# eora-ai/torchok

Hardware: AMD Instinct MI355X
Metric: images/sec (node) ResNet-50 224px bs256/GPU; step p50 ms (higher is better)
Workload: dtype bf16

## Files before the change

### torchok_amd/csrc/pw_gemm.hip

```cpp
#include "pw_gemm.h"
#include <stdlib.h>

namespace {

constexpr int BK = 64;
constexpr int BM = 128;

__device__ __forceinline__ int fw_swz(int n) {
  return ((0x78 >> (((n >> 3) & 3) << 1)) & 3) | (((n >> 1) & 1) << 2);
}

struct PwDiv { uint32_t mul, shift; };
PwDiv make_pwdiv(uint32_t d) {
  PwDiv f = {0, 0};
  if (d <= 1) return f;
  uint32_t l = 0;
  while ((1ull << l) < d) ++l;
  f.mul = (uint32_t)((((1ull << 32) * ((1ull << l) - d)) / d) + 1);
  f.shift = l;
  return f;
}
__device__ __forceinline__ uint32_t pwdiv(uint32_t n, PwDiv f) { return (uint32_t)(((uint64_t)__umulhi(n, f.mul) + n) >> f.shift); }

__device__ __forceinline__ u32x4 lds_read16(uint32_t addr) {
  u32x4 v;
  asm volatile("ds_read_b128 %0, %1" : "=v"(v) : "v"(addr));
  return v;
}
__device__ __forceinline__ uint32_t lds_read_u8(uint32_t addr) {
  uint32_t v;
  asm volatile("ds_read_u8 %0, %1" : "=v"(v) : "v"(addr));
  return v;
}

template <int BN, bool BNEP>
__global__ __launch_bounds__(256, BN == 64 ? 2 : 1) void pw_gemm_ring_kernel(PwArgs a, uint32_t x_bytes, uint32_t w_bytes,
                                                                             uint32_t y_bytes, uint32_t m_bytes, int KT,
                                                                             int SPT, uint32_t e1_bytes, PwDiv fd_hw, PwDiv fd_w,
                                                                             uint32_t x2_bytes, uint32_t w2_bytes, int KT1) {
  constexpr int NT = 256;
  constexpr int WGN = BN / 64;
  constexpr int WGM = (NT / 64) / WGN;
  constexpr int MT = BM / (WGM * 16);
  constexpr int RSTEP = NT / 8;
  constexpr int AROWS = BM / RSTEP;
  constexpr int WROWS = BN / RSTEP;
  constexpr int A_BYTES = BM * BK * 2;
  constexpr int W_BYTES = BN * BK * 2;
  constexpr int MK_BYTES = BN == 64 ? 1024 : 4096;
  constexpr int STAGE = A_BYTES + W_BYTES + MK_BYTES;
  constexpr int LOADS = AROWS + WROWS + 1;
  constexpr int NST = 3;

  extern __shared__ __attribute__((aligned(16))) char smem[];
  typedef __attribute__((address_space(3))) char lds_char;
  typedef __attribute__((address_space(3))) void lds_void;
  const uint32_t lds_base = (uint32_t)(size_t)(lds_char*)smem;

  const int tid = threadIdx.x;
  const int lane = tid & 63;
  const int wv = tid >> 6;
  const int wn = wv % WGN;
  const int wm = wv / WGN;
  const int kc = tid & 7;
  const int lrow = tid >> 3;
  const int kcA = kc ^ (lrow & 7);
  const int kcW = kc ^ fw_swz(lrow);
  const int wave_u = __builtin_amdgcn_readfirstlane(tid >> 6);

  const __amdgpu_buffer_rsrc_t xsrd = __builtin_amdgcn_make_buffer_rsrc((void*)a.x, 0, x_bytes, 0x00020000);
  const __amdgpu_buffer_rsrc_t wsrd = __builtin_amdgcn_make_buffer_rsrc((void*)a.w, 0, w_bytes, 0x00020000);
  const __amdgpu_buffer_rsrc_t x2srd = __builtin_amdgcn_make_buffer_rsrc((void*)(a.x2 ? a.x2 : a.x), 0, a.x2 ? x2_bytes : 0, 0x00020000);
  const __amdgpu_buffer_rsrc_t w2srd = __builtin_amdgcn_make_buffer_rsrc((void*)(a.w2 ? a.w2 : a.w), 0, a.w2 ? w2_bytes : 0, 0x00020000);
  const __amdgpu_buffer_rsrc_t e1srd = __builtin_amdgcn_make_buffer_rsrc((void*)(a.e1 ? a.e1 : a.x), 0, a.e1 ? e1_bytes : 0, 0x00020000);
  const __amdgpu_buffer_rsrc_t e2srd = __builtin_amdgcn_make_buffer_rsrc((void*)(a.e2 ? a.e2 : a.x), 0, a.e2 ? y_bytes : 0, 0x00020000);
  const __amdgpu_buffer_rsrc_t msrd =
      __builtin_amdgcn_make_buffer_rsrc((void*)(a.mask_in ? (const void*)a.mask_in : (const void*)a.x), 0, a.mask_in ? m_bytes : 0, 0x00020000);

  const int xcd = blockIdx.x & 7, jx = blockIdx.x >> 3;
  const int bn_fixed = jx % a.gridN, jm = jx / a.gridN;
  const int S8 = (gridDim.x >> 3) / a.gridN;
  const int sweep = 8 * S8;
  const int n0 = bn_fixed * BN;
  const int it0 = xcd * S8 + jm;
  const int ntiles = it0 < a.gridM ? (a.gridM - it0 + sweep - 1) / sweep : 0;
  const int total = ntiles * SPT;
  const int nE1 = a.e1 != nullptr ? 1 : 0;
  const int mask_cols = a.N >> 3;

  int itL = it0, ksL = 0;
  auto issue = [&](int slot) {
    char* Adst = smem + slot * STAGE + wave_u * 1024;
    char* Wdst = smem + slot * STAGE + A_BYTES + wave_u * 1024;
    char* Mdst = smem + slot * STAGE + A_BYTES + W_BYTES + wave_u * (MK_BYTES / 4);
    const bool live = itL < a.gridM;
    const int m0 = itL * BM;
    const bool kstage = ksL < KT;
    const bool last = ksL == SPT - 1;
    if (kstage) {
      const bool second = ksL >= KT1;
      const int kl = second ? ksL - KT1 : ksL;
      const int Cc = second ? a.C2 : a.C;
      const __amdgpu_buffer_rsrc_t xs = second ? x2srd : xsrd;
      const __amdgpu_buffer_rsrc_t ws = second ? w2srd : wsrd;
      const int kcol = kl * BK + kcA * 8;
#pragma unroll
      for (int i = 0; i < AROWS; ++i) {
        const int m = m0 + lrow + RSTEP * i;
        uint32_t off = (live && m < a.M && kcol < Cc) ? (uint32_t)(m * Cc + kcol) * 2u : 0xFFFFFFF0u;
        asm volatile("" : "+v"(off));
        __builtin_amdgcn_raw_ptr_buffer_load_lds(xs, (lds_void*)(Adst + i * (RSTEP * 128)), 16, off, 0, 0, 0);
      }
      const int wcol = kl * BK + kcW * 8;
#pragma unroll
      for (int j = 0; j < WROWS; ++j) {
        const int n = n0 + lrow + RSTEP * j;
        uint32_t off = (live && n < a.N && wcol < Cc) ? (uint32_t)(n * Cc + wcol) * 2u : 0xFFFFFFF0u;
        asm volatile("" : "+v"(off));
        __builtin_amdgcn_raw_ptr_buffer_load_lds(ws, (lds_void*)(Wdst + j * (RSTEP * 128)), 16, off, 0, 0, 0);
      }
    } else {
      const bool first_e = (ksL - KT) == 0 && nE1;
      const __amdgpu_buffer_rsrc_t esrd = first_e ? e1srd : e2srd;
      const bool sub = first_e && a.e1_sub;
      auto erow = [&](int m, int n, bool ok) -> uint32_t {
        if (!ok) return 0xFFFFFFF0u;
        if (sub) {
          const uint32_t b = pwdiv((uint32_t)m, fd_hw);
          const uint32_t rem = (uint32_t)m - b * (uint32_t)(a.sub_H * a.sub_W);
          const uint32_t h = pwdiv(rem, fd_w);
          const uint32_t w = rem - h * (uint32_t)a.sub_W;
          if ((h | w) & 1u) return 0xFFFFFFF0u;
          const uint32_t ph = (uint32_t)(a.sub_H + 1) >> 1, pw = (uint32_t)(a.sub_W + 1) >> 1;
          return (((b * ph + (h >> 1)) * pw + (w >> 1)) * (uint32_t)a.N + (uint32_t)n) * 2u;
        }
        return (uint32_t)(m * a.N + n) * 2u;
      };
#pragma unroll
      for (int i = 0; i < AROWS; ++i) {
        const int m = m0 + lrow + RSTEP * i;
        const int n = n0 + kcA * 8;
        uint32_t off = erow(m, n, live && m < a.M && n < a.N);
        asm volatile("" : "+v"(off));
        __builtin_amdgcn_raw_ptr_buffer_load_lds(esrd, (lds_void*)(Adst + i * (RSTEP * 128)), 16, off, 0, 0, 0);
      }
#pragma unroll
      for (int j = 0; j < WROWS; ++j) {
        const int m = m0 + lrow + RSTEP * j;
        const int n = n0 + 64 + kcA * 8;
        uint32_t off = erow(m, n, BN == 128 && live && m < a.M && n < a.N);
        asm volatile("" : "+v"(off));
        __builtin_amdgcn_raw_ptr_buffer_load_lds(esrd, (lds_void*)(Wdst + j * (RSTEP * 128)), 16, off, 0, 0, 0);
      }
    }
    {
      uint32_t off = 0xFFFFFFF0u;
      if (BN == 64) {
        const int row = tid >> 1;
        if (live && last && a.mask_in != nullptr && m0 + row < a.M) off = (uint32_t)((m0 + row) * mask_cols + (n0 >> 3) + (tid & 1) * 4);
        asm volatile("" : "+v"(off));
        __builtin_amdgcn_raw_ptr_buffer_load_lds(msrd, (lds_void*)Mdst, 4, off, 0, 0, 0);
      } else {
        if (live && last && a.mask_in != nullptr && tid < BM && m0 + tid < a.M) off = (uint32_t)((m0 + tid) * mask_cols + (n0 >> 3));
        asm volatile("" : "+v"(off));
        __builtin_amdgcn_raw_ptr_buffer_load_lds(msrd, (lds_void*)Mdst, 16, off, 0, 0, 0);
      }
    }
    if (++ksL == SPT) { ksL = 0; itL += sweep; }
  };

  const int sl = lane >> 4;
  const int li = lane & 15;
  const int wrow0 = wn * 64 + (li >> 2) * 8 + (li & 3);
  const int wswz = fw_swz(wrow0);
  const int arow0 = wm * (MT * 16) + li;
  const int aswz = li & 7;

  float s1[16], s2[16];
#pragma unroll
  for (int c = 0; c < 16; ++c) { s1[c] = 0.f; s2[c] = 0.f; }
  float esc[16], esh[16];
  if (BNEP) {
#pragma unroll
    for (int c = 0; c < 16; ++c) {
      const int n = n0 + wn * 64 + sl * 8 + (c >> 3) * 32 + (c & 7);
      esc[c] = n < a.N ? a.ep_scale[n] : 0.f;
      esh[c] = n < a.N ? a.ep_shift[n] : 0.f;
    }
  }
  float bia[16];
#pragma unroll
  for (int c = 0; c < 16; ++c) {
    const int n = n0 + wn * 64 + sl * 8 + (c >> 3) * 32 + (c & 7);
    bia[c] = (a.bias != nullptr && n < a.N) ? a.bias[n] : 0.f;
  }

  f32x4 acc[4][MT];
  auto zero_acc = [&]() {
#pragma unroll
    for (int t = 0; t < 4; ++t)
#pragma unroll
      for (int mt = 0; mt < MT; ++mt) acc[t][mt] = (f32x4){0.f, 0.f, 0.f, 0.f};
  };

  auto compute = [&](uint32_t sb) {
    const uint32_t Ab = sb, Wb = sb + A_BYTES;
    u32x4 wf[2][4], af[2][MT];
#pragma unroll
    for (int kk = 0; kk < 2; ++kk) {
      const int s = sl + 4 * kk;
#pragma unroll
      for (int t = 0; t < 4; ++t) wf[kk][t] = lds_read16(Wb + (wrow0 + (t >> 1) * 32 + (t & 1) * 4) * 128 + ((s ^ wswz) << 4));
#pragma unroll
      for (int mt = 0; mt < MT; ++mt) af[kk][mt] = lds_read16(Ab + (arow0 + mt * 16) * 128 + ((s ^ aswz) << 4));
    }
    asm volatile("s_waitcnt lgkmcnt(%0)" ::"n"(4 + MT) : "memory");
    __builtin_amdgcn_sched_barrier(0);
#pragma unroll
    for (int t = 0; t < 4; ++t)
#pragma unroll
      for (int mt = 0; mt < MT; ++mt)
        acc[t][mt] = __builtin_amdgcn_mfma_f32_16x16x32_bf16(__builtin_bit_cast(bf16x8, wf[0][t]), __builtin_bit_cast(bf16x8, af[0][mt]),
                                                             acc[t][mt], 0, 0, 0);
    __builtin_amdgcn_sched_barrier(0);
    asm volatile("s_waitcnt lgkmcnt(0)" ::: "memory");
    __builtin_amdgcn_sched_barrier(0);
#pragma unroll
    for (int t = 0; t < 4; ++t)
#pragma unroll
      for (int mt = 0; mt < MT; ++mt)
        acc[t][mt] = __builtin_amdgcn_mfma_f32_16x16x32_bf16(__builtin_bit_cast(bf16x8, wf[1][t]), __builtin_bit_cast(bf16x8, af[1][mt]),
                                                             acc[t][mt], 0, 0, 0);
  };

  auto etile = [&](uint32_t sb, bf16x8 (&dst)[MT][2]) {
    u32x4 raw[MT][2];
#pragma unroll
    for (int mt = 0; mt < MT; ++mt)
#pragma unroll
      for (int half = 0; half < 2; ++half)
        raw[mt][half] = lds_read16(sb + wn * A_BYTES + (arow0 + mt * 16) * 128 + (((sl + 4 * half) ^ aswz) << 4));
    asm volatile("s_waitcnt lgkmcnt(0)" ::: "memory");
    __builtin_amdgcn_sched_barrier(0);
#pragma unroll
    for (int mt = 0; mt < MT; ++mt)
#pragma unroll
      for (int half = 0; half < 2; ++half) dst[mt][half] = __builtin_bit_cast(bf16x8, raw[mt][half]);
  };

  auto add_e1 = [&](uint32_t sb) {
    bf16x8 ev[MT][2];
    etile(sb, ev);
#pragma unroll
    for (int mt = 0; mt < MT; ++mt)
#pragma unroll
      for (int half = 0; half < 2; ++half)
#pragma unroll
        for (int e = 0; e < 8; ++e) acc[half * 2 + (e >> 2)][mt][e & 3] += bf2f(ev[mt][half][e]);
  };

  auto epilogue = [&](int it, uint32_t sb) {
    const int m0 = it * BM;
    const int nb = n0 + wn * 64 + sl * 8;
    bf16x8 ev[MT][2];
    const bool need_tile = BNEP ? (a.e1 != nullptr) : (a.e2 != nullptr);
    if (need_tile) etile(sb, ev);
    uint32_t mbits[MT][2];
    if (a.mask_in != nullptr) {
#pragma unroll
      for (int mt = 0; mt < MT; ++mt)
#pragma unroll
        for (int half = 0; half < 2; ++half)
          mbits[mt][half] = lds_read_u8(sb + A_BYTES + W_BYTES + (arow0 + mt * 16) * (BN / 8) + wn * 8 + sl + half * 4);
      asm volatile("s_waitcnt lgkmcnt(0)" ::: "memory");
      __builtin_amdgcn_sched_barrier(0);
    }
#pragma unroll
    for (int mt = 0; mt < MT; ++mt) {
      const int m = m0 + arow0 + mt * 16;
      if (m >= a.M) continue;
      bf16* yp = a.y + (size_t)m * a.N + nb;
#pragma unroll
      for (int half = 0; half < 2; ++half) {
        if (nb + half * 32 + 8 > a.N) continue;
        float v[8];
#pragma unroll
        for (int e = 0; e < 8; ++e) v[e] = acc[half * 2 + (e >> 2)][mt][e & 3] + bia[half * 8 + e];
        bf16x8 o;
#pragma unroll
        for (int e = 0; e < 8; ++e) o[e] = f2bf(v[e]);
        const size_t eoff = (size_t)m * a.N + nb + half * 32;
        if (BNEP) {
          unsigned bits = 0;
#pragma unroll
          for (int e = 0; e < 8; ++e) {
            float z = fmaf(v[e], esc[half * 8 + e], esh[half * 8 + e]);
            if (a.e1 != nullptr) z += bf2f(ev[mt][half][e]);
            if (a.ep_relu) z = fmaxf(z, 0.f);
            o[e] = f2bf(z);
            bits |= (bf2f(o[e]) > 0.f ? 1u : 0u) << e;
          }
          if (a.mask_out != nullptr) a.mask_out[eoff >> 3] = (uint8_t)bits;
        }
        if (a.mask_store) {
          const unsigned bits = mbits[mt][half];
#pragma unroll
          for (int e = 0; e < 8; ++e) {
            if (!((bits >> e) & 1u)) o[e] = (bf16)0.f;
            s1[half * 8 + e] += bf2f(o[e]);
          }
        }
        stg16(yp + half * 32, o);
        if (a.stats != nullptr && !a.mask_store) {
          if (a.e2 != nullptr) {
            const unsigned bits = a.mask_in != nullptr ? mbits[mt][half] : 0xffu;
#pragma unroll
            for (int e = 0; e < 8; ++e) {
              const float dz = ((bits >> e) & 1u) ? bf2f(o[e]) : 0.f;
              s1[half * 8 + e] += dz;
              s2[half * 8 + e] = fmaf(dz, bf2f(ev[mt][half][e]), s2[half * 8 + e]);
            }
          } else {
#pragma unroll
            for (int e = 0; e < 8; ++e) {
              const float r = bf2f(o[e]);
              s1[half * 8 + e] += r;
              s2[half * 8 + e] = fmaf(r, r, s2[half * 8 + e]);
            }
          }
        }
      }
    }
  };

  zero_acc();
  issue(0);
  issue(1);
  int cur = 0, nxt = 2;
  int itC = it0, ksC = 0;
  for (int s = 0; s < total; ++s) {
    asm volatile("s_waitcnt vmcnt(%0) lgkmcnt(0)" ::"n"(LOADS) : "memory");
    __builtin_amdgcn_s_barrier();
    issue(nxt);
    const uint32_t sb = lds_base + cur * STAGE;
    if (ksC < KT) {
      compute(sb);
    } else if (!BNEP && a.accumulate && ksC == KT) {
      add_e1(sb);
    }
    if (ksC == SPT - 1) {
      epilogue(itC, sb);
      zero_acc();
      ksC = 0;
      itC += sweep;
    } else {
      ++ksC;
    }
    cur = cur == NST - 1 ? 0 : cur + 1;
    nxt = nxt == NST - 1 ? 0 : nxt + 1;
  }
  asm volatile("s_waitcnt vmcnt(0) lgkmcnt(0)" ::: "memory");

  if (a.stats != nullptr) {
    __syncthreads();
    float* red = reinterpret_cast<float*>(smem);
#pragma unroll
    for (int step = 0; step < 4; ++step) {
      const int off = 8 >> step;
      const int cnt = 8 >> step;
      const bool up = (li & off) != 0;
#pragma unroll
      for (int j = 0; j < cnt; ++j) {
        const float send1 = up ? s1[j] : s1[j + cnt];
        const float send2 = up ? s2[j] : s2[j + cnt];
        const float keep1 = up ? s1[j + cnt] : s1[j];
        const float keep2 = up ? s2[j + cnt] : s2[j];
        s1[j] = keep1 + __shfl_xor(send1, off, 64);
        s2[j] = keep2 + __shfl_xor(send2, off, 64);
      }
    }
    const int nl = wn * 64 + (li >> 3) * 32 + sl * 8 + (li & 7);
    red[(0 * WGM + wm) * BN + nl] = s1[0];
    red[(1 * WGM + wm) * BN + nl] = s2[0];
    __syncthreads();
    if (tid < 2 * BN) {
      const int which = tid / BN;
      const int c = tid - which * BN;
      float t = 0.f;
#pragma unroll
      for (int w_ = 0; w_ < WGM; ++w_) t += red[(which * WGM + w_) * BN + c];
      const int row = xcd * S8 + jm;
      const int n = n0 + c;
      if (n < a.N) a.stats[((size_t)which * a.stat_rows + row) * a.N + n] = t;
    }
  }
}

template <int BN, bool BNEP>
int launch_ring(const PwArgs& a, hipStream_t st) {
  constexpr int STAGE = BM * BK * 2 + BN * BK * 2 + (BN == 64 ? 1024 : 4096);
  constexpr int smem = 3 * STAGE;
  static const bool attr_set = [&] {
    (void)hipFuncSetAttribute(reinterpret_cast<const void*>(&pw_gemm_ring_kernel<BN, BNEP>),
                              hipFuncAttributeMaxDynamicSharedMemorySize, smem);
    return true;
  }();
  (void)attr_set;
  const int KT1 = tok_cdiv(a.C, BK);
  const int KT = KT1 + (a.x2 != nullptr ? tok_cdiv(a.C2, BK) : 0);
  const int SPT = KT + (a.e1 ? 1 : 0) + (a.e2 ? 1 : 0);
  const unsigned long long xb = (unsigned long long)a.M * a.C * 2, wb = (unsigned long long)a.N * a.C * 2,
                           yb = (unsigned long long)a.M * a.N * 2, mb = (unsigned long long)a.M * (a.N / 8);
  if (xb >= 0xFFFFFFF0ull || wb >= 0xFFFFFFF0ull || yb >= 0xFFFFFFF0ull) return 1;
  const unsigned long long x2b = a.x2 ? (unsigned long long)a.M * a.C2 * 2 : 0, w2b = a.x2 ? (unsigned long long)a.N * a.C2 * 2 : 0;
  if (x2b >= 0xFFFFFFF0ull) return 1;
  unsigned long long e1b = yb;
  PwDiv fd_hw = {0, 0}, fd_w = {0, 0};
  if (a.e1_sub) {
    const unsigned long long hw = (unsigned long long)a.sub_H * a.sub_W;
    e1b = (unsigned long long)(a.M / hw) * ((a.sub_H + 1) / 2) * ((a.sub_W + 1) / 2) * a.N * 2;
    fd_hw = make_pwdiv((uint32_t)hw);
    fd_w = make_pwdiv((uint32_t)a.sub_W);
  }
  const int grid = pw_ring_grid(BN, a.gridM, a.gridN);
  hipLaunchKernelGGL((pw_gemm_ring_kernel<BN, BNEP>), dim3(grid), dim3(256), smem, st, a, (uint32_t)xb, (uint32_t)wb, (uint32_t)yb,
                     (uint32_t)mb, KT, SPT, (uint32_t)e1b, fd_hw, fd_w, (uint32_t)x2b, (uint32_t)w2b, KT1);
  return 0;
}

}

int pw_ring_grid(int bn_tile, int gridM, int gridN) {
  const int unit = 8 * gridN;
  int G = 256 * (bn_tile == 64 ? 2 : 1);
  const long long need = (long long)gridM * gridN;
  if (need < G) G = (int)((need + unit - 1) / unit) * unit;
  G = G / unit * unit;
  if (G < unit) G = unit;
  return G;
}

int pw_ring_launch(const PwArgs& a, int bn_tile, hipStream_t st) {
  if (a.C % 8 != 0 || a.N % 8 != 0) return 1;
  if (a.mask_in != nullptr && a.N % 64 != 0) return 1;
  if (a.accumulate && a.e1 == nullptr) return 1;
  if ((a.x2 == nullptr) != (a.w2 == nullptr) || (a.x2 != nullptr && (a.C2 <= 0 || a.C2 % 8 != 0))) return -1;
  if (a.e1_sub && (!a.accumulate || a.ep_scale != nullptr || a.sub_H <= 0 || a.sub_W <= 0 ||
                   a.M % (a.sub_H * a.sub_W) != 0)) return -1;
  const bool bnep = a.ep_scale != nullptr;
  if (bn_tile == 64) return bnep ? launch_ring<64, true>(a, st) : launch_ring<64, false>(a, st);
  if (bnep) return 1;
  return launch_ring<128, false>(a, st);
}
```

### torchok_amd/csrc/conv_wgrad.hip

```cpp
#include "tok_common.h"
#include "conv_common.h"
#include <type_traits>
#include <stdlib.h>

namespace {

struct WgradArgs {
  const bf16* x;
  const bf16* dy;
  float* ws;
  int H, W, C, K, R, S, P, Q, stride, pad;
  int M, PQ, HW, Ktot;
  int tilesN, tilesK, splitM, mchunk;
  uint32_t x_bytes, dy_bytes;
  uint32_t pq_mul, pq_shift, q_mul, q_shift;
  float* cs;
  int cs_cols;
  int adv_q, adv_p;
  size_t cs_stride, ws_stride;
};

__device__ __forceinline__ uint32_t magic_div(uint32_t n, uint32_t mul, uint32_t shift) {
  return (uint32_t)(((uint64_t)__umulhi(n, mul) + n) >> shift);
}
// ... 883 lines not shown
    asm volatile("s_waitcnt vmcnt(%0) lgkmcnt(0)" ::"n"((NST - 2) * LOADS) : "memory");
    __builtin_amdgcn_s_barrier();
    __builtin_amdgcn_sched_barrier(0);
    const int rd2 = rd == NST - 1 ? 0 : rd + 1;
    bf16x8 af[NT];
#pragma unroll
    for (int i = 0; i < NT; ++i) af[i] = __builtin_bit_cast(bf16x8, (u32x4){ycur[i][0][0], ycur[i][0][1], ycur[i][1][0], ycur[i][1][1]});
#pragma unroll
    for (int j = 0; j < KTL; ++j) {
      if (W0 * KTL + j < NTILES) {
        const bf16x8 bfr = __builtin_bit_cast(bf16x8, (u32x4){xb[j][0][0], xb[j][0][1], xb[j][1][0], xb[j][1][1]});
#pragma unroll
        for (int i = 0; i < NT; ++i) acc[i][j] = __builtin_amdgcn_mfma_f32_16x16x32_bf16(af[i], bfr, acc[i][j], 0, 0, 0);
      }
      if (j < LOADS) issue_piece(wr, j);
      if (j == 0) advance();
      if (j >= 1 && (j - 1) * 2 < NT) { read_y(rd, (j - 1) * 2, ynxt); if ((j - 1) * 2 + 1 < NT) read_y(rd, (j - 1) * 2 + 1, ynxt); }
      read_x(tb, j, xb);
#pragma unroll
      for (int k = 0; k < 3; ++k)
        if (last_j(k) == j) bases_tap(rd2, k, tb);
      __builtin_amdgcn_sched_barrier(0);
    }
    rd = rd2;
    wr = wr == NST - 1 ? 0 : wr + 1;
  };
  for (int st = 0; st < steps; st += 2) {
    body(yA, yB);
    if (st + 1 < steps) body(yB, yA);
  }
  asm volatile("s_waitcnt vmcnt(0) lgkmcnt(0)" ::: "memory");

  int lane2;
  asm volatile("v_mbcnt_lo_u32_b32 %0, -1, 0\n\tv_mbcnt_hi_u32_b32 %0, -1, %0" : "=v"(lane2));
  const int g = lane2 >> 4, li = lane2 & 15;
  float* out = a.ws + (size_t)split * a.K * a.Ktot;
#pragma unroll
  for (int j = 0; j < KTL; ++j) {
    const int J = W0 * KTL + j;
    if (J >= NTILES) continue;
    const int cin = ct * TC + (J % CT) * 16 + li;
    const int kcol = (J / CT) * a.C + cin;
#pragma unroll
    for (int i = 0; i < NT; ++i)
#pragma unroll
      for (int r = 0; r < 4; ++r) {
        const int n = tn * TN + i * 16 + g * 4 + r;
        if (n < a.K && cin < a.C) out[(size_t)n * a.Ktot + kcol] = acc[i][j][r];
      }
  }
  };
  if (wv == 0) run(std::integral_constant<int, 0>{});
  else if (wv == 1) run(std::integral_constant<int, 1>{});
  else if (wv == 2) run(std::integral_constant<int, 2>{});
  else run(std::integral_constant<int, 3>{});
}

__global__ void wgrad_reduce_kernel(const float* __restrict__ ws, float* __restrict__ dw, int splitM,
                                    int k_real, int R, int S, int c_real, int K, int S_pad,
                                    int C_pad, int accumulate) {
  const size_t total = (size_t)k_real * R * S * c_real;
  const size_t slab = (size_t)K * R * S_pad * C_pad;
  for (size_t i = (size_t)blockIdx.x * blockDim.x + threadIdx.x; i < total;
       i += (size_t)gridDim.x * blockDim.x) {
    const int c = (int)(i % c_real);
    size_t rest = i / c_real;
    const int s = (int)(rest % S);
    rest /= S;
    const int r = (int)(rest % R);
    const int k = (int)(rest / R);
    const size_t src = (((size_t)k * R + r) * S_pad + s) * C_pad + c;
    float t = 0.f;
    for (int sp = 0; sp < splitM; sp += 8) {
      float v[8];
#pragma unroll
      for (int u = 0; u < 8; ++u) v[u] = ws[(size_t)(sp + u < splitM ? sp + u : splitM - 1) * slab + src];
#pragma unroll
      for (int u = 0; u < 8; ++u) t += sp + u < splitM ? v[u] : 0.f;
    }
    dw[i] = accumulate ? dw[i] + t : t;
  }
}

template <int U>
__device__ __forceinline__ void reduce_slabs(const float* __restrict__ ws, size_t stride, size_t i, int row, int splitM, float4& t) {
  for (int sp = row; sp < splitM; sp += 16 * U) {
    float4 v[U];
#pragma unroll
    for (int u = 0; u < U; ++u) {
      const int su = sp + 16 * u;
      v[u] = reinterpret_cast<const float4*>(ws + (size_t)(su < splitM ? su : splitM - 1) * stride)[i];
    }
#pragma unroll
    for (int u = 0; u < U; ++u) {
      if (sp + 16 * u < splitM) { t.x += v[u].x; t.y += v[u].y; t.z += v[u].z; t.w += v[u].w; }
    }
  }
}

__global__ __launch_bounds__(256) void wgrad_reduce_flat_kernel(const float* __restrict__ ws, float* __restrict__ dw,
                                                                int splitM, size_t slab, int accumulate, size_t stride,
                                                                float* __restrict__ extra, int extra_n, int extra_pad,
                                                                int extra_acc) {
  __shared__ float4 red[16][16];
  const int col = threadIdx.x & 15, row = threadIdx.x >> 4;
  const size_t m4 = slab >> 2;
  const size_t n4 = m4 + (extra != nullptr ? (size_t)(extra_pad >> 2) : 0);
  for (size_t base = (size_t)blockIdx.x * 16; base < n4; base += (size_t)gridDim.x * 16) {
    const size_t i = base + col;
    float4 t = {0.f, 0.f, 0.f, 0.f};
    if (i < n4) {
      if (splitM > 64) reduce_slabs<8>(ws, stride, i, row, splitM, t);
      else if (splitM > 32) reduce_slabs<4>(ws, stride, i, row, splitM, t);
      else if (splitM > 16) reduce_slabs<2>(ws, stride, i, row, splitM, t);
      else if (row < splitM) {
        const float4 v = reinterpret_cast<const float4*>(ws + (size_t)row * stride)[i];
        t.x += v.x; t.y += v.y; t.z += v.z; t.w += v.w;
      }
    }
    red[row][col] = t;
    __syncthreads();
    for (int s_ = 8; s_ > 0; s_ >>= 1) {
      if (row < s_) {
        const float4 o = red[row + s_][col];
        float4 m = red[row][col];
        m.x += o.x; m.y += o.y; m.z += o.z; m.w += o.w;
        red[row][col] = m;
      }
      __syncthreads();
    }
    if (row == 0 && i < m4) {
      float4 r = red[0][col];
      if (accumulate) {
        const float4 o = reinterpret_cast<const float4*>(dw)[i];
        r.x += o.x; r.y += o.y; r.z += o.z; r.w += o.w;
      }
      reinterpret_cast<float4*>(dw)[i] = r;
    } else if (row == 0 && i < n4) {
      const float4 r = red[0][col];
      const float rv[4] = {r.x, r.y, r.z, r.w};
      const int e0 = (int)(i - m4) * 4;
#pragma unroll
      for (int e = 0; e < 4; ++e)
        if (e0 + e < extra_n) extra[e0 + e] = extra_acc ? extra[e0 + e] + rv[e] : rv[e];
    }
    __syncthreads();
  }
}

struct Plan {
  int TN, TK, tilesN, tilesK, splitM, mchunk, MS;
  bool ring;
  bool taps;
};

static int taps_target() {
  static const int v = [] { const char* e = getenv("TOK_WGRAD_TAPS_WGS"); return (int)(e ? atoi(e) : 256); }();
  return v;
}

static int ring_target() {
  static const int v = [] { const char* e = getenv("TOK_WGRAD_WGS"); return (int)(e ? atoi(e) : 0); }();
  return v;
}

Plan make_plan(const tok_conv_desc* d) {
  Plan p;
  const int Ktot = d->r * d->s_pad * d->c;
  const long long M = (long long)d->n * d->p * d->q;
  p.taps = false;
  const bool same3 = d->r == 3 && d->s == 3 && d->s_pad == 3 && d->stride == 1 && d->pad == 1 &&
                     (unsigned long long)d->n * d->h * d->w * d->c * 2 < 0x40000000ull &&
                     (unsigned long long)d->n * d->p * d->q * d->k * 2 < 0x40000000ull;
  const bool w64 = d->c % 64 == 0 && d->k % 64 == 0;
  const bool w48 = !w64 && d->c % 48 == 0 && d->k % 48 == 0 && same3;
  if (d->c != 4 && (w64 || w48) && d->r == 3 && d->s == 3 && d->s_pad == 3) {
    p.taps = true; p.ring = false;
    p.TN = w64 ? 64 : 48; p.TK = p.TN; p.MS = 32;
    p.tilesN = tok_cdiv(d->k, p.TN);
    p.tilesK = tok_cdiv(d->c, p.TN);
    const int tiles = p.tilesN * p.tilesK;
    long long split = (taps_target() + tiles - 1) / tiles;
    const long long max_split = (M + 8 * 32 - 1) / (8 * 32);
    if (split > max_split) split = max_split;
    if (split > 512) split = 512;
    if (split < 1) split = 1;
    long long chunk = (M + split - 1) / split;
    chunk = ((chunk + 31) / 32) * 32;
    p.mchunk = (int)chunk;
    p.splitM = (int)((M + chunk - 1) / chunk);
    return p;
  }
  p.ring = d->c != 4 && d->r == 1 && d->s == 1 && d->stride == 1 && d->pad == 0;
  if (p.ring) {
    p.MS = 32;
    if (d->k <= 64) { p.TN = 64; p.TK = Ktot >= 256 ? 256 : (Ktot >= 128 ? 128 : 64); }
    else if (Ktot <= 64) { p.TK = 64; p.TN = d->k >= 256 ? 256 : 128; }
    else { p.TN = 128; p.TK = 128; }
    static const int big = [] { const char* e = getenv("TOK_WGRAD_256"); return (int)(e ? atoi(e) : 1); }();
    if (big && d->r == 1 && d->s == 1 && d->stride == 1 && d->pad == 0 && d->k >= 256 && Ktot >= 256 && M >= (big >= 2 ? 8192 : 200000) &&
        (long long)tok_cdiv(d->k, 256) * tok_cdiv(Ktot, 256) * 65536 * 2 <= (long long)d->k * Ktot * 3) {
      p.TN = 256; p.TK = 256;
    }
    p.tilesN = tok_cdiv(d->k, p.TN);
    p.tilesK = tok_cdiv(Ktot, p.TK);
    const int tiles = p.tilesN * p.tilesK;
    const int stage = 32 * (p.TN + p.TK) * 2;
    const int per_cu = (160 * 1024) / (3 * stage);
    static const int long_target = [] { const char* e = getenv("TOK_WGRAD_WGS_LONG"); return (int)(e ? atoi(e) : 0); }();
    const int target = (long_target > 0 && M >= 100000) ? long_target
                       : ring_target() > 0 ? ring_target() : 256 * (per_cu > 2 ? 2 : per_cu);
    long long split = (target + tiles - 1) / tiles;
    const long long max_split = (M + 8 * 32 - 1) / (8 * 32);
    if (split > max_split) split = max_split;
    if (split > 512) split = 512;
    if (split < 1) split = 1;
    long long chunk = (M + split - 1) / split;
    chunk = ((chunk + 31) / 32) * 32;
    p.mchunk = (int)chunk;
    p.splitM = (int)((M + chunk - 1) / chunk);
    return p;
  }
  p.TN = d->k >= 128 ? 128 : 64;
  p.TK = Ktot >= 128 ? 128 : 64;
  p.tilesN = tok_cdiv(d->k, p.TN);
  p.tilesK = tok_cdiv(Ktot, p.TK);
  const int tiles = p.tilesN * p.tilesK;
  static const int tb_target = [] { const char* e = getenv("TOK_WGRAD_2BUF_WGS"); return (int)(e ? atoi(e) : 1024); }();
  long long split = (tb_target + tiles - 1) / tiles;
  p.MS = (M >= 100000 && p.TN == 128 && p.TK == 128) ? 64 : 32;
// ... 107 lines not shown
  a.H = d->h; a.W = d->w; a.C = d->c; a.K = d->k; a.R = d->r; a.S = d->s_pad; a.P = d->p; a.Q = d->q;
  a.stride = d->stride; a.pad = d->pad;
  a.M = d->n * d->p * d->q; a.PQ = d->p * d->q; a.HW = d->h * d->w;
  make_magic((uint32_t)a.PQ, a.pq_mul, a.pq_shift);
  make_magic((uint32_t)d->q, a.q_mul, a.q_shift);
  a.adv_q = 32 % d->q; a.adv_p = (32 / d->q) % d->p;
  a.Ktot = d->r * d->s_pad * d->c;
  a.tilesN = p.tilesN; a.tilesK = p.tilesK; a.splitM = p.splitM; a.mchunk = p.mchunk;
  const size_t slab_f = (size_t)d->k * d->r * d->s_pad * d->c;
  const int cs_pad = (k_real + 3) / 4 * 4;
  const bool cs_inline = dbias != nullptr && flat && !direct;
  a.ws_stride = cs_inline ? slab_f + cs_pad : slab_f;
  a.cs = dbias ? (cs_inline ? (float*)ws + slab_f : (float*)((char*)ws + tok_conv_wgrad_ws_bytes(d))) : nullptr;
  a.cs_stride = cs_inline ? a.ws_stride : (size_t)k_real;
  a.cs_cols = k_real;
  {
    const unsigned long long xb = (unsigned long long)d->n * d->h * d->w * d->c * 2;
    const unsigned long long yb = (unsigned long long)a.M * d->k * 2;
    TOK_CHECK_ARG(xb < 0xFFFFFFF0ull && yb < 0xFFFFFFF0ull, "tok_conv_wgrad: tensors of 4 GiB or more are not supported");
    a.x_bytes = (uint32_t)xb; a.dy_bytes = (uint32_t)yb;
  }
  hipStream_t st = tok_stream(stream);
  const bool c4 = d->c == 4;
  if (c4 && dbias == nullptr && stem_wgrad_serves(d)) {
    stem_wgrad_launch(d, x, dy, a.ws, p.splitM, st);
  } else
  if (p.taps) {
    constexpr int smem = 3 * 10 * 32 * 128;
    static const bool attr_set = [&] {
      (void)hipFuncSetAttribute(reinterpret_cast<const void*>(&conv_wgrad_taps_kernel<0>),
                                hipFuncAttributeMaxDynamicSharedMemorySize, smem);
      return true;
    }();
    (void)attr_set;
    const bool same = a.stride == 1 && a.pad == 1 && a.P == a.H && a.Q == a.W && a.x_bytes < 0x40000000u && a.dy_bytes < 0x40000000u;
    if (same) {
      constexpr int smem_p = 3 * (32 * 128 + 128 * 128);
      static const bool attr_p = [&] {
        (void)hipFuncSetAttribute(reinterpret_cast<const void*>(&conv_wgrad_winp_kernel<4, 3, 9>), hipFuncAttributeMaxDynamicSharedMemorySize, smem_p);
        (void)hipFuncSetAttribute(reinterpret_cast<const void*>(&conv_wgrad_winp_kernel<3, 3, 7>), hipFuncAttributeMaxDynamicSharedMemorySize, smem_p);
        return true;
      }();
      (void)attr_p;
      const dim3 gw(a.tilesN * a.tilesK * a.splitM);
      if (p.TN == 48) hipLaunchKernelGGL((conv_wgrad_winp_kernel<3, 3, 7>), gw, dim3(256), smem_p, st, a);
      else hipLaunchKernelGGL((conv_wgrad_winp_kernel<4, 3, 9>), gw, dim3(256), smem_p, st, a);
    } else {
      hipLaunchKernelGGL((conv_wgrad_taps_kernel<0>), dim3(a.tilesN * a.tilesK * a.splitM), dim3(256), smem, st, a);
    }
  } else if (p.ring) {
    if (p.TN == 256 && p.TK == 256) {
      constexpr int smem8 = 3 * 32 * (256 + 256) * 2;
      static const bool attr8 = [] {
        (void)hipFuncSetAttribute(reinterpret_cast<const void*>(&conv_wgrad_ring8_kernel<256, 256>),
                                  hipFuncAttributeMaxDynamicSharedMemorySize, smem8);
        return true;
      }();
      (void)attr8;
      hipLaunchKernelGGL((conv_wgrad_ring8_kernel<256, 256>), dim3(a.tilesN * a.tilesK * a.splitM), dim3(512), smem8, st, a);
    }
    else if (p.TN == 64 && p.TK == 64) launch_ring<64, 64>(a, st);
    else if (p.TN == 64 && p.TK == 128) launch_ring<64, 128>(a, st);
    else if (p.TN == 64 && p.TK == 256) launch_ring<64, 256>(a, st);
    else if (p.TN == 128 && p.TK == 64) launch_ring<128, 64>(a, st);
    else if (p.TN == 256 && p.TK == 64) launch_ring<256, 64>(a, st);
    else launch_ring<128, 128>(a, st);
  } else if (p.TN == 128 && p.TK == 128) {
    if (c4) launch_wgrad<128, 128, true>(a, st, p.MS); else launch_wgrad<128, 128, false>(a, st, p.MS);
  } else if (p.TN == 128) {
    if (c4) launch_wgrad<128, 64, true>(a, st, p.MS); else launch_wgrad<128, 64, false>(a, st, p.MS);
  } else if (p.TK == 128) {
    if (c4) launch_wgrad<64, 128, true>(a, st, p.MS); else launch_wgrad<64, 128, false>(a, st, p.MS);
  } else {
    if (c4) launch_wgrad<64, 64, true>(a, st, p.MS); else launch_wgrad<64, 64, false>(a, st, p.MS);
  }
  TOK_CHECK_LAUNCH("tok_conv_wgrad");
  if (dbias != nullptr && !cs_inline) {
    if (int e = tok_colsum_f32(a.cs, p.splitM, k_real, dbias, bias_accumulate, stream)) return e;
  }
  if (direct) return TOK_OK;
  if (flat) {
    if (tok_dbg_skip(2)) return TOK_OK;
    const size_t slab = (size_t)d->k * d->r * d->s * d->c;
    const size_t nb = (slab / 4 + 15) / 16;
    hipLaunchKernelGGL(wgrad_reduce_flat_kernel, dim3((int)(nb < 4096 ? nb : 4096)), dim3(256), 0, st,
                       (const float*)ws, dw, p.splitM, slab, accumulate, cs_inline ? a.ws_stride : slab,
                       cs_inline ? dbias : (float*)nullptr, k_real, cs_inline ? cs_pad : 0, bias_accumulate);
    TOK_CHECK_LAUNCH("tok_conv_wgrad(reduce)");
    return TOK_OK;
  }
  const size_t total = (size_t)k_real * d->r * d->s * c_real;
  const int blocks = (int)((total + 255) / 256 < 2048 ? (total + 255) / 256 : 2048);
  hipLaunchKernelGGL(wgrad_reduce_kernel, dim3(blocks), dim3(256), 0, st, (const float*)ws, dw,
                     p.splitM, k_real, d->r, d->s, c_real, d->k, d->s_pad, d->c, accumulate);
  TOK_CHECK_LAUNCH("tok_conv_wgrad(reduce)");
  return TOK_OK;
}
}
```

Baseline: 14380.

## Add weight-stationary register mode for small-K pointwise GEMM tiles

For 64-wide tiles with C at most 128 and no second input, each thread loads its weight fragments once from global memory into registers, and per-stage weight loads into LDS are skipped. This cuts LDS traffic, LDS reads per k-step and shared-memory footprint, which may raise occupancy for small-channel 1x1 convolutions. The cost is extra VGPR pressure from holding up to two k-slabs of weights, and statistics and sum code paths are compiled out for the BN-epilogue variant.

```diff
diff --git a/torchok_amd/csrc/pw_gemm.hip b/torchok_amd/csrc/pw_gemm.hip
--- a/torchok_amd/csrc/pw_gemm.hip
+++ b/torchok_amd/csrc/pw_gemm.hip
@@ -33,7 +33,7 @@
   return v;
 }
 
-template <int BN, bool BNEP>
+template <int BN, bool BNEP, int WS>
 __global__ __launch_bounds__(256, BN == 64 ? 2 : 1) void pw_gemm_ring_kernel(PwArgs a, uint32_t x_bytes, uint32_t w_bytes,
                                                                              uint32_t y_bytes, uint32_t m_bytes, int KT,
                                                                              int SPT, uint32_t e1_bytes, PwDiv fd_hw, PwDiv fd_w,
@@ -48,9 +48,12 @@
   constexpr int A_BYTES = BM * BK * 2;
   constexpr int W_BYTES = BN * BK * 2;
   constexpr int MK_BYTES = BN == 64 ? 1024 : 4096;
-  constexpr int STAGE = A_BYTES + W_BYTES + MK_BYTES;
-  constexpr int LOADS = AROWS + WROWS + 1;
+  static_assert(WS == 0 || BN == 64, "weight-stationary mode: 64-wide tiles");
+  constexpr int MK_OFF = A_BYTES + (WS ? 0 : W_BYTES);
+  constexpr int STAGE = MK_OFF + MK_BYTES;
+  constexpr int LOADS = AROWS + (WS ? 0 : WROWS) + 1;
   constexpr int NST = 3;
+  constexpr bool SUMS = !(BNEP && WS != 0);
 
   extern __shared__ __attribute__((aligned(16))) char smem[];
   typedef __attribute__((address_space(3))) char lds_char;
@@ -92,7 +95,7 @@
   auto issue = [&](int slot) {
     char* Adst = smem + slot * STAGE + wave_u * 1024;
     char* Wdst = smem + slot * STAGE + A_BYTES + wave_u * 1024;
-    char* Mdst = smem + slot * STAGE + A_BYTES + W_BYTES + wave_u * (MK_BYTES / 4);
+    char* Mdst = smem + slot * STAGE + MK_OFF + wave_u * (MK_BYTES / 4);
     const bool live = itL < a.gridM;
     const int m0 = itL * BM;
     const bool kstage = ksL < KT;
@@ -111,13 +114,15 @@
         asm volatile("" : "+v"(off));
         __builtin_amdgcn_raw_ptr_buffer_load_lds(xs, (lds_void*)(Adst + i * (RSTEP * 128)), 16, off, 0, 0, 0);
       }
-      const int wcol = kl * BK + kcW * 8;
-#pragma unroll
-      for (int j = 0; j < WROWS; ++j) {
-        const int n = n0 + lrow + RSTEP * j;
-        uint32_t off = (live && n < a.N && wcol < Cc) ? (uint32_t)(n * Cc + wcol) * 2u : 0xFFFFFFF0u;
-        asm volatile("" : "+v"(off));
-        __builtin_amdgcn_raw_ptr_buffer_load_lds(ws, (lds_void*)(Wdst + j * (RSTEP * 128)), 16, off, 0, 0, 0);
+      if constexpr (WS == 0) {
+        const int wcol = kl * BK + kcW * 8;
+#pragma unroll
+        for (int j = 0; j < WROWS; ++j) {
+          const int n = n0 + lrow + RSTEP * j;
+          uint32_t off = (live && n < a.N && wcol < Cc) ? (uint32_t)(n * Cc + wcol) * 2u : 0xFFFFFFF0u;
+          asm volatile("" : "+v"(off));
+          __builtin_amdgcn_raw_ptr_buffer_load_lds(ws, (lds_void*)(Wdst + j * (RSTEP * 128)), 16, off, 0, 0, 0);
+        }
       }
     } else {
       const bool first_e = (ksL - KT) == 0 && nE1;
@@ -144,13 +149,15 @@
         asm volatile("" : "+v"(off));
         __builtin_amdgcn_raw_ptr_buffer_load_lds(esrd, (lds_void*)(Adst + i * (RSTEP * 128)), 16, off, 0, 0, 0);
       }
-#pragma unroll
-      for (int j = 0; j < WROWS; ++j) {
-        const int m = m0 + lrow + RSTEP * j;
-        const int n = n0 + 64 + kcA * 8;
-        uint32_t off = erow(m, n, BN == 128 && live && m < a.M && n < a.N);
-        asm volatile("" : "+v"(off));
-        __builtin_amdgcn_raw_ptr_buffer_load_lds(esrd, (lds_void*)(Wdst + j * (RSTEP * 128)), 16, off, 0, 0, 0);
+      if constexpr (WS == 0) {
+#pragma unroll
+        for (int j = 0; j < WROWS; ++j) {
+          const int m = m0 + lrow + RSTEP * j;
+          const int n = n0 + 64 + kcA * 8;
+          uint32_t off = erow(m, n, BN == 128 && live && m < a.M && n < a.N);
+          asm volatile("" : "+v"(off));
+          __builtin_amdgcn_raw_ptr_buffer_load_lds(esrd, (lds_void*)(Wdst + j * (RSTEP * 128)), 16, off, 0, 0, 0);
+        }
       }
     }
     {
@@ -203,18 +210,44 @@
       for (int mt = 0; mt < MT; ++mt) acc[t][mt] = (f32x4){0.f, 0.f, 0.f, 0.f};
   };
 
-  auto compute = [&](uint32_t sb) {
+  u32x4 wst[WS ? WS : 1][2][4];
+  if constexpr (WS != 0) {
+#pragma unroll
+    for (int ks = 0; ks < WS; ++ks)
+#pragma unroll
+      for (int kk = 0; kk < 2; ++kk)
+#pragma unroll
+        for (int t = 0; t < 4; ++t) {
+          const int n = n0 + wrow0 + (t >> 1) * 32 + (t & 1) * 4;
+          const int k = ks * BK + (sl + 4 * kk) * 8;
+          const bool ok = n < a.N && k < a.C;
+          const u32x4* src = reinterpret_cast<const u32x4*>(a.w + (ok ? (size_t)n * a.C + k : 0));
+          const u32x4 v = *src;
+          wst[ks][kk][t] = ok ? v : (u32x4){0u, 0u, 0u, 0u};
+        }
+#pragma unroll
+    for (int ks = 0; ks < WS; ++ks)
+#pragma unroll
+      for (int kk = 0; kk < 2; ++kk)
+#pragma unroll
+        for (int t = 0; t < 4; ++t) asm volatile("" : "+v"(wst[ks][kk][t]));
+  }
+
+  auto compute = [&](uint32_t sb, const u32x4 (&wreg)[2][4]) {
     const uint32_t Ab = sb, Wb = sb + A_BYTES;
     u32x4 wf[2][4], af[2][MT];
 #pragma unroll
     for (int kk = 0; kk < 2; ++kk) {
       const int s = sl + 4 * kk;
 #pragma unroll
-      for (int t = 0; t < 4; ++t) wf[kk][t] = lds_read16(Wb + (wrow0 + (t >> 1) * 32 + (t & 1) * 4) * 128 + ((s ^ wswz) << 4));
+      for (int t = 0; t < 4; ++t) {
+        if constexpr (WS == 0) wf[kk][t] = lds_read16(Wb + (wrow0 + (t >> 1) * 32 + (t & 1) * 4) * 128 + ((s ^ wswz) << 4));
+        else wf[kk][t] = wreg[kk][t];
+      }
 #pragma unroll
       for (int mt = 0; mt < MT; ++mt) af[kk][mt] = lds_read16(Ab + (arow0 + mt * 16) * 128 + ((s ^ aswz) << 4));
     }
-    asm volatile("s_waitcnt lgkmcnt(%0)" ::"n"(4 + MT) : "memory");
+    asm volatile("s_waitcnt lgkmcnt(%0)" ::"n"((WS ? 0 : 4) + MT) : "memory");
     __builtin_amdgcn_sched_barrier(0);
 #pragma unroll
     for (int t = 0; t < 4; ++t)
@@ -271,7 +304,7 @@
       for (int mt = 0; mt < MT; ++mt)
 #pragma unroll
         for (int half = 0; half < 2; ++half)
-          mbits[mt][half] = lds_read_u8(sb + A_BYTES + W_BYTES + (arow0 + mt * 16) * (BN / 8) + wn * 8 + sl + half * 4);
+          mbits[mt][half] = lds_read_u8(sb + MK_OFF + (arow0 + mt * 16) * (BN / 8) + wn * 8 + sl + half * 4);
       asm volatile("s_waitcnt lgkmcnt(0)" ::: "memory");
       __builtin_amdgcn_sched_barrier(0);
     }
@@ -302,7 +335,7 @@
           }
           if (a.mask_out != nullptr) a.mask_out[eoff >> 3] = (uint8_t)bits;
         }
-        if (a.mask_store) {
+        if (SUMS && a.mask_store) {
           const unsigned bits = mbits[mt][half];
 #pragma unroll
           for (int e = 0; e < 8; ++e) {
@@ -311,7 +344,7 @@
           }
         }
         stg16(yp + half * 32, o);
-        if (a.stats != nullptr && !a.mask_store) {
+        if (SUMS && a.stats != nullptr && !a.mask_store) {
           if (a.e2 != nullptr) {
             const unsigned bits = a.mask_in != nullptr ? mbits[mt][half] : 0xffu;
 #pragma unroll
@@ -344,7 +377,12 @@
     issue(nxt);
     const uint32_t sb = lds_base + cur * STAGE;
     if (ksC < KT) {
-      compute(sb);
+      if constexpr (WS == 2) {
+        if (ksC == 0) compute(sb, wst[0]);
+        else compute(sb, wst[1]);
+      } else {
+        compute(sb, wst[0]);
+      }
     } else if (!BNEP && a.accumulate && ksC == KT) {
       add_e1(sb);
     }
@@ -361,7 +399,7 @@
   }
   asm volatile("s_waitcnt vmcnt(0) lgkmcnt(0)" ::: "memory");
 
-  if (a.stats != nullptr) {
+  if (SUMS && a.stats != nullptr) {
     __syncthreads();
     float* red = reinterpret_cast<float*>(smem);
 #pragma unroll
@@ -396,12 +434,12 @@
   }
 }
 
-template <int BN, bool BNEP>
+template <int BN, bool BNEP, int WS>
 int launch_ring(const PwArgs& a, hipStream_t st) {
-  constexpr int STAGE = BM * BK * 2 + BN * BK * 2 + (BN == 64 ? 1024 : 4096);
+  constexpr int STAGE = BM * BK * 2 + (WS ? 0 : BN * BK * 2) + (BN == 64 ? 1024 : 4096);
   constexpr int smem = 3 * STAGE;
   static const bool attr_set = [&] {
-    (void)hipFuncSetAttribute(reinterpret_cast<const void*>(&pw_gemm_ring_kernel<BN, BNEP>),
+    (void)hipFuncSetAttribute(reinterpret_cast<const void*>(&pw_gemm_ring_kernel<BN, BNEP, WS>),
                               hipFuncAttributeMaxDynamicSharedMemorySize, smem);
     return true;
   }();
@@ -423,7 +461,7 @@
     fd_w = make_pwdiv((uint32_t)a.sub_W);
   }
   const int grid = pw_ring_grid(BN, a.gridM, a.gridN);
-  hipLaunchKernelGGL((pw_gemm_ring_kernel<BN, BNEP>), dim3(grid), dim3(256), smem, st, a, (uint32_t)xb, (uint32_t)wb, (uint32_t)yb,
+  hipLaunchKernelGGL((pw_gemm_ring_kernel<BN, BNEP, WS>), dim3(grid), dim3(256), smem, st, a, (uint32_t)xb, (uint32_t)wb, (uint32_t)yb,
                      (uint32_t)mb, KT, SPT, (uint32_t)e1b, fd_hw, fd_w, (uint32_t)x2b, (uint32_t)w2b, KT1);
   return 0;
 }
@@ -448,7 +486,14 @@
   if (a.e1_sub && (!a.accumulate || a.ep_scale != nullptr || a.sub_H <= 0 || a.sub_W <= 0 ||
                    a.M % (a.sub_H * a.sub_W) != 0)) return -1;
   const bool bnep = a.ep_scale != nullptr;
-  if (bn_tile == 64) return bnep ? launch_ring<64, true>(a, st) : launch_ring<64, false>(a, st);
+  if (bn_tile == 64) {
+    const bool ws_ok = a.x2 == nullptr && a.C <= 2 * BK && ((uintptr_t)a.w & 15) == 0 &&
+                       !(bnep && (a.stats != nullptr || a.mask_store));
+    const int ws = ws_ok ? tok_cdiv(a.C, BK) : 0;
+    if (ws == 1) return bnep ? launch_ring<64, true, 1>(a, st) : launch_ring<64, false, 1>(a, st);
+    if (ws == 2) return bnep ? launch_ring<64, true, 2>(a, st) : launch_ring<64, false, 2>(a, st);
+    return bnep ? launch_ring<64, true, 0>(a, st) : launch_ring<64, false, 0>(a, st);
+  }
   if (bnep) return 1;
-  return launch_ring<128, false>(a, st);
-}
+  return launch_ring<128, false, 0>(a, st);
+}
```

New measurement: 14430 (median of 6 runs). About the same (+0.3%).

## Replace LDS tree split-K reduction with register-folded wavefront shuffle reduction

Applied to the files above, without the earlier changes.

Swaps the flat split-M reduction kernel, which used a 16x16 shared-memory tree with block-wide barriers, for a templated fold kernel. Each thread accumulates several slabs in registers, folds them locally, and combines groups across the wavefront with shuffles, with no LDS and no __syncthreads. A host heuristic picks the group count, per-thread slab classes and unroll from splitM and output size so that small outputs still launch enough waves. This removes barrier and LDS traffic from the reduction step but adds many template instantiations and somewhat intricate index logic.

```diff
diff --git a/torchok_amd/csrc/conv_wgrad.hip b/torchok_amd/csrc/conv_wgrad.hip
--- a/torchok_amd/csrc/conv_wgrad.hip
+++ b/torchok_amd/csrc/conv_wgrad.hip
@@ -989,70 +989,109 @@
   }
 }
 
-template <int U>
-__device__ __forceinline__ void reduce_slabs(const float* __restrict__ ws, size_t stride, size_t i, int row, int splitM, float4& t) {
-  for (int sp = row; sp < splitM; sp += 16 * U) {
-    float4 v[U];
-#pragma unroll
-    for (int u = 0; u < U; ++u) {
-      const int su = sp + 16 * u;
-      v[u] = reinterpret_cast<const float4*>(ws + (size_t)(su < splitM ? su : splitM - 1) * stride)[i];
-    }
-#pragma unroll
-    for (int u = 0; u < U; ++u) {
-      if (sp + 16 * u < splitM) { t.x += v[u].x; t.y += v[u].y; t.z += v[u].z; t.w += v[u].w; }
-    }
-  }
-}
-
-__global__ __launch_bounds__(256) void wgrad_reduce_flat_kernel(const float* __restrict__ ws, float* __restrict__ dw,
-                                                                int splitM, size_t slab, int accumulate, size_t stride,
-                                                                float* __restrict__ extra, int extra_n, int extra_pad,
-                                                                int extra_acc) {
-  __shared__ float4 red[16][16];
-  const int col = threadIdx.x & 15, row = threadIdx.x >> 4;
+template <int G, int C, int U>
+__global__ __launch_bounds__(256) void wgrad_fold_kernel(const float* __restrict__ ws, float* __restrict__ dw, int splitM,
+                                                         size_t slab, int accumulate, size_t stride, float* __restrict__ extra,
+                                                         int extra_n, int extra_pad, int extra_acc) {
+  static_assert(G * C <= 16 && (U == 1 || G * C == 16), "wgrad_fold_kernel: bad shape");
+  constexpr int W = 64 / G;
+  const int lane = threadIdx.x & 63, g = lane / W;
   const size_t m4 = slab >> 2;
   const size_t n4 = m4 + (extra != nullptr ? (size_t)(extra_pad >> 2) : 0);
-  for (size_t base = (size_t)blockIdx.x * 16; base < n4; base += (size_t)gridDim.x * 16) {
-    const size_t i = base + col;
-    float4 t = {0.f, 0.f, 0.f, 0.f};
-    if (i < n4) {
-      if (splitM > 64) reduce_slabs<8>(ws, stride, i, row, splitM, t);
-      else if (splitM > 32) reduce_slabs<4>(ws, stride, i, row, splitM, t);
-      else if (splitM > 16) reduce_slabs<2>(ws, stride, i, row, splitM, t);
-      else if (row < splitM) {
-        const float4 v = reinterpret_cast<const float4*>(ws + (size_t)row * stride)[i];
-        t.x += v.x; t.y += v.y; t.z += v.z; t.w += v.w;
-      }
-    }
-    red[row][col] = t;
-    __syncthreads();
-    for (int s_ = 8; s_ > 0; s_ >>= 1) {
-      if (row < s_) {
-        const float4 o = red[row + s_][col];
-        float4 m = red[row][col];
-        m.x += o.x; m.y += o.y; m.z += o.z; m.w += o.w;
-        red[row][col] = m;
-      }
-      __syncthreads();
-    }
-    if (row == 0 && i < m4) {
-      float4 r = red[0][col];
-      if (accumulate) {
-        const float4 o = reinterpret_cast<const float4*>(dw)[i];
-        r.x += o.x; r.y += o.y; r.z += o.z; r.w += o.w;
-      }
-      reinterpret_cast<float4*>(dw)[i] = r;
-    } else if (row == 0 && i < n4) {
-      const float4 r = red[0][col];
-      const float rv[4] = {r.x, r.y, r.z, r.w};
-      const int e0 = (int)(i - m4) * 4;
-#pragma unroll
-      for (int e = 0; e < 4; ++e)
-        if (e0 + e < extra_n) extra[e0 + e] = extra_acc ? extra[e0 + e] + rv[e] : rv[e];
-    }
-    __syncthreads();
-  }
+  const size_t i = ((size_t)blockIdx.x * 4 + (threadIdx.x >> 6)) * W + lane % W;
+  const bool live = i < n4;
+  const float4* src = reinterpret_cast<const float4*>(ws) + (live ? i : 0);
+  const size_t stride4 = stride >> 2;
+  float4 t[C];
+#pragma unroll
+  for (int c = 0; c < C; ++c) t[c] = {0.f, 0.f, 0.f, 0.f};
+  for (int s0 = 0; s0 < splitM; s0 += 16 * U) {
+    float4 v[U][C];
+#pragma unroll
+    for (int u = 0; u < U; ++u)
+#pragma unroll
+      for (int c = 0; c < C; ++c) {
+        const int s = s0 + 16 * u + G * c + g;
+        v[u][c] = src[(size_t)(s < splitM ? s : splitM - 1) * stride4];
+      }
+#pragma unroll
+    for (int u = 0; u < U; ++u)
+#pragma unroll
+      for (int c = 0; c < C; ++c)
+        if (s0 + 16 * u + G * c + g < splitM) { t[c].x += v[u][c].x; t[c].y += v[u][c].y; t[c].z += v[u][c].z; t[c].w += v[u][c].w; }
+  }
+#pragma unroll
+  for (int step = 8; step >= G; step >>= 1) {
+    const int cs = step / G;
+#pragma unroll
+    for (int c = 0; c < cs; ++c)
+      if (c + cs < C) { t[c].x += t[c + cs].x; t[c].y += t[c + cs].y; t[c].z += t[c + cs].z; t[c].w += t[c + cs].w; }
+  }
+#pragma unroll
+  for (int step = G / 2; step > 0; step >>= 1) {
+    float4 o;
+    o.x = __shfl_down(t[0].x, step * W); o.y = __shfl_down(t[0].y, step * W);
+    o.z = __shfl_down(t[0].z, step * W); o.w = __shfl_down(t[0].w, step * W);
+    if (g < step) { t[0].x += o.x; t[0].y += o.y; t[0].z += o.z; t[0].w += o.w; }
+  }
+  if (g != 0 || !live) return;
+  float4 r = t[0];
+  if (i < m4) {
+    if (accumulate) {
+      const float4 o = reinterpret_cast<const float4*>(dw)[i];
+      r.x += o.x; r.y += o.y; r.z += o.z; r.w += o.w;
+    }
+    reinterpret_cast<float4*>(dw)[i] = r;
+  } else {
+    const float rv[4] = {r.x, r.y, r.z, r.w};
+    const int e0 = (int)(i - m4) * 4;
+#pragma unroll
+    for (int e = 0; e < 4; ++e)
+      if (e0 + e < extra_n) extra[e0 + e] = extra_acc ? extra[e0 + e] + rv[e] : rv[e];
+  }
+}
+
+struct FoldArgs {
+  const float* ws; float* dw; int splitM; size_t slab; int accumulate; size_t stride;
+  float* extra; int extra_n, extra_pad, extra_acc;
+};
+
+template <int G, int C, int U = 1>
+void fold_launch_u(int u, const FoldArgs& f, hipStream_t st) {
+  if constexpr (G * C == 16 && U < G) {
+    if (u > U) { fold_launch_u<G, C, U * 2>(u, f, st); return; }
+  }
+  const size_t n4 = (f.slab >> 2) + (f.extra != nullptr ? (size_t)(f.extra_pad >> 2) : 0);
+  const size_t waves = (n4 + 64 / G - 1) / (64 / G);
+  hipLaunchKernelGGL((wgrad_fold_kernel<G, C, U>), dim3((unsigned)((waves + 3) / 4)), dim3(256), 0, st, f.ws, f.dw, f.splitM,
+                     f.slab, f.accumulate, f.stride, f.extra, f.extra_n, f.extra_pad, f.extra_acc);
+}
+
+template <int G = 1>
+void fold_launch(int g, int classes, int u, const FoldArgs& f, hipStream_t st) {
+  if constexpr (G < 16) {
+    if (g > G) { fold_launch<G * 2>(g, classes, u, f, st); return; }
+  }
+  switch (classes / G) {
+    case 1: if constexpr (G >= 2) { fold_launch_u<G, 1>(u, f, st); } return;
+    case 2: if constexpr (G <= 8) { fold_launch_u<G, 2>(u, f, st); } return;
+    case 4: if constexpr (G <= 4) { fold_launch_u<G, 4>(u, f, st); } return;
+    case 8: if constexpr (G <= 2) { fold_launch_u<G, 8>(u, f, st); } return;
+    default: if constexpr (G == 1) { fold_launch_u<1, 16>(u, f, st); } return;
+  }
+}
+
+void fold(const FoldArgs& f, hipStream_t st) {
+  constexpr int gmax = 16;
+  constexpr size_t wmin = 1024;
+  int classes = 2;
+  while (classes < 16 && classes < f.splitM) classes *= 2;
+  const size_t n4 = (f.slab >> 2) + (f.extra != nullptr ? (size_t)(f.extra_pad >> 2) : 0);
+  int g = 1;
+  while (g < gmax && g < classes && (n4 * g + 63) / 64 < wmin) g *= 2;
+  int u = 1;
+  while (u < g && 16 * u < f.splitM) u *= 2;
+  fold_launch<1>(g, classes, u, f, st);
 }
 
 struct Plan {
@@ -1326,10 +1365,8 @@
   if (flat) {
     if (tok_dbg_skip(2)) return TOK_OK;
     const size_t slab = (size_t)d->k * d->r * d->s * d->c;
-    const size_t nb = (slab / 4 + 15) / 16;
-    hipLaunchKernelGGL(wgrad_reduce_flat_kernel, dim3((int)(nb < 4096 ? nb : 4096)), dim3(256), 0, st,
-                       (const float*)ws, dw, p.splitM, slab, accumulate, cs_inline ? a.ws_stride : slab,
-                       cs_inline ? dbias : (float*)nullptr, k_real, cs_inline ? cs_pad : 0, bias_accumulate);
+    fold({(const float*)ws, dw, p.splitM, slab, accumulate, cs_inline ? a.ws_stride : slab,
+          cs_inline ? dbias : (float*)nullptr, k_real, cs_inline ? cs_pad : 0, bias_accumulate}, st);
     TOK_CHECK_LAUNCH("tok_conv_wgrad(reduce)");
     return TOK_OK;
   }
```

Measured after the change: 14550 before, 14650 after (median of 6 runs). No clear change (+0.7%).
